# facebookresearch/param

Measured on AMD Instinct MI355X. Metric: EmbeddingBag lookups/s + achieved HBM GB/s; all-to-all bus-BW at 1/2/4/8 GPU, higher is better.
Workload: dtype f32

## Files before the change

param_amd/csrc/capi.hip:

```cpp
#include <atomic>
#include <cstdio>
#include <cstdlib>
#include <string>

#include "common.h"

namespace pm {
hipError_t launch_embbag_fwd_qrows(const KParams& p, int bits, int out_dtype, int max_dim, int unroll, hipStream_t stream);
hipError_t launch_embbag_fwd_qmixed(const KParams& p, const int32_t* table_bits, int out_dtype, int max_dim, int unroll, hipStream_t stream);
}

namespace {

thread_local std::string g_last_error;

std::atomic<int> g_unroll{0};
std::atomic<int> g_bags_per_block{0};
std::atomic<int> g_xcd_affine{-1};
std::atomic<int> g_nt_loads{-1};
std::atomic<int> g_stage_out{-1};
std::atomic<int> g_flat_target{-1};
std::atomic<int> g_flat_grid{-1};
constexpr int kDefaultRowPolicy = 3;

int fail(int code, const std::string& msg) {
    g_last_error = msg;
    return code;
}

int hip_fail(hipError_t rc, const char* what) {
    return fail(PM_ERR_HIP, std::string(what) + ": " + hipGetErrorString(rc));
}

const pm::FwdEnv& fwd_env() {
    static const pm::FwdEnv e = [] {
        auto num = [](const char* name, int dflt) { const char* v = getenv(name); return v ? atoi(v) : dflt; };
        pm::FwdEnv r;
        const char* st = getenv("PARAM_AMD_FWD_STAGE");
        r.stage = (st && st[0] == '0') ? 0 : 1;
        r.flat = num("PARAM_AMD_FWD_FLAT", r.flat);
        r.flat_maxl = num("PARAM_AMD_FLAT_MAXL", r.flat_maxl);
        r.flat_target = num("PARAM_AMD_FLAT_TARGET", r.flat_target);
        r.flat_bags = num("PARAM_AMD_FLAT_BAGS", r.flat_bags);
        r.tile_major = num("PARAM_AMD_FWD_TILE_MAJOR", r.tile_major);
        r.flat_compact = num("PARAM_AMD_FLAT_COMPACT", r.flat_compact);
        return r;
    }();
    return e;
}

pm::PlanKnobs current_knobs() {
    constexpr auto relaxed = std::memory_order_relaxed;
    pm::TuningSetters s;
    s.unroll = g_unroll.load(relaxed);
    s.bags_per_block = g_bags_per_block.load(relaxed);
    s.xcd_affine = g_xcd_affine.load(relaxed);
    s.nt_loads = g_nt_loads.load(relaxed);
    s.stage_out = g_stage_out.load(relaxed);
    s.flat_grid = g_flat_grid.load(relaxed);
    s.flat_target = g_flat_target.load(relaxed);
    return pm::resolve_knobs(s, fwd_env());
}

bool dtype_is_weight(int d) { return d == PM_F32 || d == PM_BF16 || d == PM_F16; }

const char* const kNoSortRecorded = "no sort has been recorded for this workspace";

enum class PlanKind { base, forward, quantized, padded, padded16 };

int validate_request(const pm_embbag_batch* op, int elem_dtype, const pm::PlanKnobs& knobs, pm::PlanShape* shape = nullptr);
void fill_params(const pm_embbag_batch* op, const pm::LaunchPlan& plan, pm::KParams& p);

pm::LaunchPlan plan_of(const pm_embbag_batch& op, const pm::PlanShape& shape, const pm::PlanKnobs& knobs, PlanKind kind) {
    return kind == PlanKind::forward     ? pm::plan_forward(op, shape, knobs)
           : kind == PlanKind::quantized ? pm::plan_quantized(op, shape, knobs)
           : kind == PlanKind::padded    ? pm::plan_padded(op, shape, knobs, 4)
           : kind == PlanKind::padded16  ? pm::plan_padded(op, shape, knobs, 2)
                                         : pm::plan_base(op, shape, knobs);
}

int make_params(const pm_embbag_batch* op, int elem_dtype, pm::KParams& p, PlanKind kind = PlanKind::base, int* unroll = nullptr) {
// ... 43 lines not shown
}

void fill_params(const pm_embbag_batch* op, const pm::LaunchPlan& plan, pm::KParams& p) {
    p.tables = op->tables;
    p.rows = op->rows;
    p.dims = op->dims;
    p.out_offsets = op->out_offsets;
    p.indices = op->indices;
    p.offsets = op->offsets;
    p.psw = op->per_sample_weights;
    p.io = nullptr;
    p.out_stride = op->out_stride;
    p.B = op->batch;
    p.N = op->num_indices;
    p.bag_begin = op->bag_begin;
    p.bag_count = op->bag_count;
    p.T = op->num_tables;
    p.idx64 = op->index_dtype == PM_I64 ? 1 : 0;
    p.alpha = 1.0f;
    p.gblk_shift = op->grad_block_shift > 0 ? op->grad_block_shift : 31;
    p.gblk_extra = op->grad_block_shift > 0 ? op->grad_block_extra : 0;
    p.out_bits = 0;
    p.tiles_per_table = plan.tiles_per_table;
    p.bags_per_block = plan.bags_per_block;
    p.idx_cap = plan.idx_cap;
    p.xcd_affine = plan.xcd_affine;
    p.nt_loads = plan.nt_loads;
    p.ordered = plan.ordered;
    p.stage_out = plan.stage_out;
    p.stage_bags = plan.stage_bags;
    p.flat_bags = plan.flat_bags;
    p.flat_target = plan.flat_target;
    p.flat_compact = plan.flat_compact;
}

int plan_fail(pm::PlanStatus st, const char* kind, bool sequence = false) {
    switch (st) {
        case pm::PlanStatus::ok: return PM_OK;
        case pm::PlanStatus::none:
            if (sequence)
                return fail(PM_ERR_INVALID, "pm_embseq_sort_indices has not been called for this request on this workspace (same indices / "
                                            "offsets pointers, batch and bag slice as the sort's)");
            return fail(PM_ERR_INVALID, "pm_embbag_sort_indices has not been called for this request on this workspace (same indices / "
                                        "offsets pointers, batch, bag slice and weights as the sort's)");
        case pm::PlanStatus::two_phase:
            return fail(PM_ERR_INVALID, std::string("the request was sorted for a two-phase scatter-add apply; ") + kind + " Adagrad needs "
                                        "pm_embbag_sort_indices (phases = 1)");
        case pm::PlanStatus::relabelled:
            return fail(PM_ERR_INVALID, "the sort on this workspace was relabelled by pm_embbag_sparse_grad_count (its keys hold slots, not "
                                        "rows): sort the request again");
        case pm::PlanStatus::not_complete_segmented:
            return fail(PM_ERR_UNSUPPORTED, "the sparse gradient needs the complete one-phase segmented sort: sort with pm_embbag_sort_indices "
                                            "(sort_impl 0)");
        case pm::PlanStatus::low_digit_order:
            return fail(PM_ERR_UNSUPPORTED, "the sparse gradient needs rows in ascending order within a table: sort mode 1 orders them by "
                                            "their low digit first (pm_set_sort_tuning 0, 2 or 3)");
        case pm::PlanStatus::sequence_sort:
            return fail(PM_ERR_INVALID, "the sort on this workspace is a sequence sort (pm_embseq_sort_indices: its values are lookup positions, "
                                        "not bags): only pm_embseq_bwd_sorted* may follow it; sort the request with pm_embbag_sort_indices");
        case pm::PlanStatus::pooled_sort:
            return fail(PM_ERR_INVALID, "the sort on this workspace is a pooled sort (pm_embbag_sort_indices: its values are bags, not lookup "
                                        "positions): a sequence apply needs pm_embseq_sort_indices");
        case pm::PlanStatus::already_counted:
            return fail(PM_ERR_INVALID, "pm_embbag_sparse_grad_count has been called for this sort already: sort the request again");
        default: return fail(PM_ERR_INVALID, "pm_embbag_sparse_grad needs pm_embbag_sparse_grad_count on this sort first");
    }
// ... 77 lines not shown

int pm_abi_version(void) { return PM_ABI_VERSION; }

const char* pm_build_info(void) {
    return "libparam_amd gfx950 (CDNA4, wave64) hip " __VERSION__;
}

const char* pm_last_error(void) { return g_last_error.c_str(); }

int pm_set_tuning(int32_t unroll, int32_t bags_per_block, int32_t xcd_affine, int32_t nt_loads) {
    if (unroll != 0 && unroll != 1 && unroll != 2 && unroll != 3 && unroll != 4 && unroll != 6 && unroll != 8)
        return fail(PM_ERR_INVALID, "unroll must be 0, 1, 2, 3, 4, 6 or 8");
    if (bags_per_block < 0) return fail(PM_ERR_INVALID, "bags_per_block must be >= 0");
    g_unroll.store(unroll);
    g_bags_per_block.store(bags_per_block);
    g_xcd_affine.store(xcd_affine);
    g_nt_loads.store(nt_loads);
    return PM_OK;
}

int pm_set_forward_tuning(int32_t stage_out, int32_t flat_grid, int32_t flat_target) {
    if (stage_out < -1 || stage_out > 1) return fail(PM_ERR_INVALID, "stage_out must be -1, 0 or 1");
    if (flat_grid < -1 || flat_grid > (1 << 20)) return fail(PM_ERR_INVALID, "flat_grid must be -1 (default), 0, 1 or a workgroup count up to 2^20");
    if (flat_target < -1 || flat_target == 0 || flat_target > 4096) return fail(PM_ERR_INVALID, "flat_target must be -1 (default) or 1 .. 4096");
    g_stage_out.store(stage_out);
    g_flat_grid.store(flat_grid);
    g_flat_target.store(flat_target);
    return PM_OK;
}

int pm_embbag_plan(const pm_embbag_batch* op, int32_t kind, int32_t out[12]) {
    if (kind < PM_PLAN_BASE || kind > PM_PLAN_PADDED16) return fail(PM_ERR_INVALID, "kind must be PM_PLAN_BASE .. PM_PLAN_PADDED16");
    if (!out) return fail(PM_ERR_INVALID, "out is NULL");
    static_assert(sizeof(pm::LaunchPlan) == 12 * sizeof(int32_t), "the query copies the twelve members in their order");
    const pm::PlanKnobs knobs = current_knobs();
    pm::PlanShape shape;
    const int rc = validate_request(op, op ? op->weight_dtype : -1, knobs, &shape);
    if (rc != PM_OK) return rc;
    constexpr PlanKind kinds[] = {PlanKind::base, PlanKind::forward, PlanKind::quantized, PlanKind::padded, PlanKind::padded16};
    const pm::LaunchPlan p = plan_of(*op, shape, knobs, kinds[kind]);
    const int32_t v[12] = {p.tiles_per_table, p.bags_per_block, p.idx_cap, p.xcd_affine, p.nt_loads, p.ordered,
                           p.stage_out, p.stage_bags, p.flat_bags, p.flat_target, p.flat_compact, p.unroll};
    for (int i = 0; i < 12; ++i) out[i] = v[i];
    return PM_OK;
}

int pm_embedding_gather_plan(const pm_embbag_batch* op, int64_t out[8]) {
    if (!out) return fail(PM_ERR_INVALID, "out is NULL");
    const pm::PlanKnobs knobs = current_knobs();
    const int rc = validate_request(op, op ? op->weight_dtype : -1, knobs);
    if (rc != PM_OK) return rc;
    const pm::GatherPlan g = pm::plan_gather(*op, op->weight_dtype, knobs);
    const int64_t v[8] = {g.vec, g.group_lanes, g.tile, g.col_passes, g.unroll, g.lds_borders, g.xcd_contiguous, g.grid};
    for (int i = 0; i < 8; ++i) out[i] = v[i];
    return PM_OK;
}

int pm_set_backward_tuning(int32_t sort_impl, int32_t order, int32_t xcd_affine, int32_t max_phases) {
    if (sort_impl < -1 || sort_impl > 2 || order < -1 || order > 1 || xcd_affine < -1 || xcd_affine > 1)
        return fail(PM_ERR_INVALID, "sort_impl must be -1 .. 2, order / xcd_affine -1, 0 or 1");
#ifndef PM_ALTERNATES
    if (sort_impl > 0)
        return fail(PM_ERR_UNSUPPORTED, "sort_impl 1 (rocPRIM) and 2 (round 2's LSD sort) exist in the alternates build only "
                                        "(libparam_amd_alt.so: make -C param_amd/csrc alt)");
#endif
    if (max_phases != -1 && max_phases != 1 && max_phases != 2) return fail(PM_ERR_INVALID, "max_phases must be -1, 1 or 2");
    pm::set_backward_tuning(sort_impl, order, xcd_affine, max_phases);
// ... 940 lines not shown
```

param_amd/csrc/common.h:

```cpp
#pragma once

#include <hip/hip_runtime.h>
#include <stdint.h>

#include <string>
#include <type_traits>

#include "param_amd.h"
#include "launch_plan.h"

namespace pm {

constexpr int kWave = 64;

typedef uint32_t u32x4 __attribute__((ext_vector_type(4)));
typedef float f32x4 __attribute__((ext_vector_type(4)));

#define PM_GLOBAL __attribute__((address_space(1)))
template <typename T>
__device__ __forceinline__ const PM_GLOBAL T* as_global(const void* p) { return (const PM_GLOBAL T*)(p); }
template <typename T>
__device__ __forceinline__ PM_GLOBAL T* as_global(void* p) { return (PM_GLOBAL T*)(p); }

struct KParams {
    const void* const* tables;
    const int64_t* rows;
    const int32_t* dims;
    const int64_t* out_offsets;
    const void* indices;
    const void* offsets;
    const float* psw;
    float* io;
    int64_t out_stride;
    int64_t B;
    int64_t N;
    int64_t bag_begin;
    int64_t bag_count;
    int32_t T;
    int32_t tiles_per_table;
    int32_t bags_per_block;
    int32_t idx_cap;
    int32_t idx64;
    int32_t xcd_affine;
    int32_t nt_loads;
    int32_t ordered;
    int32_t stage_out;
    int32_t stage_bags;
    int32_t out_bits;
    int32_t flat_bags;
    int32_t flat_target;
    int32_t flat_compact;
    int32_t gblk_shift;
    int64_t gblk_extra;
    float alpha;
};

__device__ __forceinline__ int64_t grad_bag_offset(int64_t bag, int64_t out_stride, int shift, int64_t extra) {
    int64_t o = bag * out_stride;
    if (__builtin_expect(extra != 0, 0)) o += (bag >> shift) * extra;
    return o;
}

__device__ __forceinline__ int64_t load_index(const void* p, int64_t i, int idx64) {
    return idx64 ? as_global<int64_t>(p)[i] : static_cast<int64_t>(as_global<int32_t>(p)[i]);
}

__device__ __forceinline__ int64_t bag_start_or_end(const KParams& p, int64_t g) {
    const int64_t TB = static_cast<int64_t>(p.T) * p.B;
    return (g < TB) ? load_index(p.offsets, g, p.idx64) : p.N;
}

__device__ __forceinline__ int xcd_contiguous_tile(int bid, int total) {
    const int q = total / kXcds, r = total % kXcds, x = bid % kXcds;
    return x * q + (x < r ? x : r) + bid / kXcds;
}

__device__ __forceinline__ void block_to_tile(const KParams& p, int& t, int& tile, int bid = blockIdx.x) {
    if (p.xcd_affine == 3) {
        const int g = xcd_contiguous_tile(bid, p.T * p.tiles_per_table);
        t = g / p.tiles_per_table;
        tile = g % p.tiles_per_table;
    } else if (p.xcd_affine == 2) {
        t = bid % p.T;
        tile = bid / p.T;
    } else if (p.xcd_affine) {
        const int xcd = bid % kXcds;
        const int slot = bid / kXcds;
        t = xcd + kXcds * (slot / p.tiles_per_table);
        tile = slot % p.tiles_per_table;
    } else {
        t = bid / p.tiles_per_table;
        tile = bid % p.tiles_per_table;
    }
}

__host__ __device__ inline size_t tile_idx_offset(int bags_per_block) {
    return (static_cast<size_t>(bags_per_block + 2) / 2 * 2) * sizeof(int64_t);
}
__host__ __device__ inline size_t tile_lds_bytes(int bags_per_block, int idx_cap, bool weighted) {
    return tile_idx_offset(bags_per_block) + static_cast<size_t>(idx_cap) * 4 * (weighted ? 2 : 1);
}

template <bool WEIGHTED>
__device__ __forceinline__ bool stage_tile_at(const KParams& p, int t, int64_t bag0, int nb, char* smem,
                                              int64_t*& s_off, int32_t*& s_idx, float*& s_w) {
    const int64_t g0 = static_cast<int64_t>(t) * p.B + bag0;

    s_off = reinterpret_cast<int64_t*>(smem);
    s_idx = reinterpret_cast<int32_t*>(smem + tile_idx_offset(p.bags_per_block));
    s_w = reinterpret_cast<float*>(s_idx + p.idx_cap);

    for (int i = threadIdx.x; i <= nb; i += kBlock) s_off[i] = bag_start_or_end(p, g0 + i);
    __syncthreads();
    const int64_t base = s_off[0];
    const int64_t cnt = s_off[nb] - base;
    const bool staged = cnt <= p.idx_cap;
    if (staged) {
        for (int i = threadIdx.x; i < static_cast<int>(cnt); i += kBlock) {
            s_idx[i] = static_cast<int32_t>(load_index(p.indices, base + i, p.idx64));
            if (WEIGHTED) s_w[i] = as_global<float>(p.psw)[base + i];
        }
        __syncthreads();
    }
    return staged;
}

// ... 259 lines not shown
```

param_amd/csrc/embbag_fwd.hip:

```cpp
#include <type_traits>

#include "common.h"
#include "fwd_elem.h"
#include "rowquant.inc"

namespace pm {
namespace {

using namespace fwd;

__device__ __forceinline__ float shfl_min(float v, int width) {
    for (int m = width / 2; m >= 1; m >>= 1) v = fminf(v, __shfl_xor(v, m, width));
    return v;
}
__device__ __forceinline__ float shfl_max(float v, int width) {
    for (int m = width / 2; m >= 1; m >>= 1) v = fmaxf(v, __shfl_xor(v, m, width));
    return v;
}

template <int BITS>
__device__ __forceinline__ void fused_rows_burst(const float* s_out, int nb, int D, uint8_t* qout, int64_t row0, int64_t rows_per_bag) {
    int gq = 4;
    while (gq * 8 < D) gq *= 2;
    const int lane = threadIdx.x % gq;
    const int c0 = lane * 4, c1 = (gq + lane) * 4;
    const bool has0 = c0 < D, has1 = c1 < D;
    const int64_t rb = rq::row_bytes(D, BITS);
    for (int r0 = 0; r0 < nb; r0 += kBlock / gq) {
        const int bg = r0 + threadIdx.x / gq;
        const bool live = bg < nb;
        const float* src = s_out + static_cast<size_t>(live ? bg : 0) * D;
        const f32x4 a = has0 ? *reinterpret_cast<const f32x4*>(src + c0) : f32x4{0, 0, 0, 0};
        const f32x4 b = has1 ? *reinterpret_cast<const f32x4*>(src + c1) : f32x4{0, 0, 0, 0};
        float mn, mx;
        rq::row_min_max(a, b, has0, has1, mn, mx);
        mn = shfl_min(mn, gq);
// ... 6 lines not shown

__device__ __forceinline__ void quantized_burst(const KParams& p, const float* s_out, int nb, int D, int64_t bag0, int64_t out_off) {
    uint8_t* qout = reinterpret_cast<uint8_t*>(p.io);
    const int64_t rows_per_bag = p.out_stride / D;
    const int64_t row0 = bag0 * rows_per_bag + out_off / D;
    switch (p.out_bits) {
        case 16: {
            typedef uint32_t u32x2 __attribute__((ext_vector_type(2)));
            const int q = D / 4;
            for (int i = threadIdx.x; i < nb * q; i += kBlock) {
                const int bg = i / q, c4 = i % q;
                const f32x4 v = *reinterpret_cast<const f32x4*>(s_out + static_cast<size_t>(bg) * D + c4 * 4);
                u32x2 o;
                o.x = rq::half_bits(v.x) | (static_cast<uint32_t>(rq::half_bits(v.y)) << 16);
                o.y = rq::half_bits(v.z) | (static_cast<uint32_t>(rq::half_bits(v.w)) << 16);
                __builtin_nontemporal_store(o, reinterpret_cast<u32x2*>(qout + (row0 + bg * rows_per_bag) * 2 * D) + c4);
            }
            break;
        }
        case 8: fused_rows_burst<8>(s_out, nb, D, qout, row0, rows_per_bag); break;
        case 4: fused_rows_burst<4>(s_out, nb, D, qout, row0, rows_per_bag); break;
        default: fused_rows_burst<2>(s_out, nb, D, qout, row0, rows_per_bag); break;
    }
}

template <typename WT, int G, int UNROLL, bool WEIGHTED, bool ORDERED, bool STAGE>
__global__ void __launch_bounds__(kBlock) embbag_fwd_kernel(const KParams p) {
    constexpr int VEC = Elem<WT>::kVec;
    constexpr int NG = kBlock / G;
    extern __shared__ __attribute__((aligned(16))) char smem[];
    __shared__ int s_next;

    int t, tile;
    block_to_tile(p, t, tile);
    if (t >= p.T) return;
    const int64_t bag0 = p.bag_begin + static_cast<int64_t>(tile) * p.bags_per_block;
    const int64_t left_bags = p.bag_begin + p.bag_count - bag0;
    const int nb = left_bags < p.bags_per_block ? static_cast<int>(left_bags) : p.bags_per_block;
    if (threadIdx.x == 0) s_next = NG;

    int64_t* s_off;
    int32_t* s_idx;
    float* s_w;
    const bool staged = stage_tile_at<WEIGHTED>(p, t, bag0, nb, smem, s_off, s_idx, s_w);
    const int64_t base = s_off[0];
    __shared__ uint16_t s_ord[ORDERED ? 1024 : 1];
    if (ORDERED) {
        if (nb <= kWave) {
            if (threadIdx.x < kWave) {
                const int i = threadIdx.x;
                int64_t len = i < nb ? s_off[i + 1] - s_off[i] : -1;
                if (len > 0x7fffffffffffLL) len = 0x7fffffffffffLL;
                uint64_t key = (static_cast<uint64_t>(len + 1) << 16) | static_cast<uint64_t>(0xffff - i);
#pragma unroll
                for (int k = 2; k <= kWave; k <<= 1) {
#pragma unroll
                    for (int j = k >> 1; j > 0; j >>= 1) {
                        const uint64_t other = __shfl_xor(key, j, kWave);
                        const bool take_max = ((i & k) == 0) == ((i & j) == 0);
                        key = take_max ? (key > other ? key : other) : (key < other ? key : other);
                    }
                }
                if (i < nb) s_ord[i] = static_cast<uint16_t>(0xffff - (key & 0xffff));
            }
        } else {
            for (int i = threadIdx.x; i < nb; i += kBlock) {
                const int64_t li = s_off[i + 1] - s_off[i];
                int rank = 0;
                for (int j = 0; j < nb; ++j) {
                    const int64_t lj = s_off[j + 1] - s_off[j];
                    rank += (lj > li) || (lj == li && j < i);
// ... 71 lines not shown
                        }
                    }
                }

                if (STAGE && stage) {
                    f32x4* o4 = reinterpret_cast<f32x4*>(s_out + static_cast<size_t>(bg) * D + c);
#pragma unroll
                    for (int k = 0; k < VEC; k += 4) o4[k / 4] = f32x4{acc[k], acc[k + 1], acc[k + 2], acc[k + 3]};
                } else {
                    f32x4* o4 = reinterpret_cast<f32x4*>(orow + c);
#pragma unroll
                    for (int k = 0; k < VEC; k += 4) {
                        f32x4 v = {acc[k], acc[k + 1], acc[k + 2], acc[k + 3]};
                        __builtin_nontemporal_store(v, o4 + k / 4);
                    }
                }
            }
        };
        if (staged) pool(std::true_type{}); else pool(std::false_type{});
        int nxt = 0;
        if (lig == 0) nxt = atomicAdd(&s_next, 1);
        slot = __shfl(nxt, 0, G);
    }
    if (STAGE && stage) {
        __syncthreads();
        if (p.out_bits == 0) {
            const int q = D / 4;
            if ((q & (q - 1)) != 0) burst_rows<false>(s_out, out_t, bag0, p.out_stride, nb, D);
            else burst_rows<true>(s_out, out_t, bag0, p.out_stride, nb, D);
        } else {
            quantized_burst(p, s_out, nb, D, bag0, p.out_offsets[t]);
        }
    }
}


__host__ __device__ inline size_t flat_tables_offset(const KParams& p, bool weighted) {
    return (tile_lds_bytes(p.bags_per_block, p.idx_cap, weighted) + static_cast<size_t>(p.stage_bags) * p.stage_out * sizeof(float) + 15) / 16 * 16;
}

template <typename WT, int G, int UNROLL, bool WEIGHTED>
__global__ void __launch_bounds__(kBlock) embbag_fwd_flat_kernel(const KParams p) {
    constexpr int VEC = Elem<WT>::kVec;
    extern __shared__ __attribute__((aligned(16))) char smem[];
    int* const s_pref = reinterpret_cast<int*>(smem + flat_tables_offset(p, WEIGHTED));
    uint16_t* const s_bags = reinterpret_cast<uint16_t*>(s_pref + p.T + 1);

    auto geometry = [&](int t, int& D, int& g, int& bags) {
        D = p.dims[t];
        g = kBlock / p.flat_bags;
        if (g < 1) g = 1;
        while (g < G && g * VEC < D) g <<= 1;
        const int NG = kBlock / g;
        const int64_t g0 = static_cast<int64_t>(t) * p.B + p.bag_begin;
        const int64_t lo = bag_start_or_end(p, g0), hi = bag_start_or_end(p, g0 + p.bag_count);
        const int64_t avg = p.bag_count > 0 ? (hi - lo + p.bag_count - 1) / p.bag_count : 1;
        bags = static_cast<int>(p.flat_target / (avg > 0 ? avg : 1));
        bags = bags > p.flat_bags ? p.flat_bags : bags;
        bags = bags / NG * NG;
        if (bags < NG) bags = NG;
    };

    auto do_tile = [&](int t, int tile, int D, int g, int bags) {
        const int NG = kBlock / g;
        const int64_t bag0 = p.bag_begin + static_cast<int64_t>(tile) * bags;
        const int64_t left_bags = p.bag_begin + p.bag_count - bag0;
// ... 106 lines not shown
                running += __shfl(v, kWave - 1, kWave);
            }
            if (threadIdx.x == 0) s_pref[0] = 0;
        }
        __syncthreads();
    }
    const int total = compact ? s_pref[p.T] : static_cast<int>(blockIdx.x) + 1;
    const int step = compact ? static_cast<int>(gridDim.x) : 1;
    for (int v = blockIdx.x; v < total; v += step) {
        int t, tile, D, g, bags;
        if (compact) {
            int lo = 0, hi = p.T;
            while (hi - lo > 1) {
                const int mid = (lo + hi) >> 1;
                if (s_pref[mid] <= v) lo = mid; else hi = mid;
            }
            t = lo;
            tile = v - s_pref[t];
            D = p.dims[t];
            g = kBlock / p.flat_bags;
            if (g < 1) g = 1;
            while (g < G && g * VEC < D) g <<= 1;
            bags = s_bags[t];
        } else {
            block_to_tile(p, t, tile);
            if (t >= p.T) return;
            geometry(t, D, g, bags);
        }
        do_tile(t, tile, D, g, bags);
        if (compact) __syncthreads();
    }
}

template <typename WT, int G, int UNROLL>
hipError_t launch_w(const KParams& p, hipStream_t stream) {
    const bool weighted = p.psw != nullptr;
    int grid = p.T * p.tiles_per_table;
    size_t lds = tile_lds_bytes(p.bags_per_block, p.idx_cap, weighted);
    if (p.flat_bags > 0) {
        lds += static_cast<size_t>(p.stage_bags) * p.stage_out * sizeof(float);
        if (p.flat_compact > 0) {
            lds = flat_tables_offset(p, weighted) + static_cast<size_t>(p.T + 1) * 4 + static_cast<size_t>(p.T) * 2;
            if (p.flat_compact < grid) grid = p.flat_compact;
        }
        dispatch_bool(weighted, [&](auto w) {
            hipLaunchKernelGGL((embbag_fwd_flat_kernel<WT, G, UNROLL, decltype(w)::value>), dim3(grid), dim3(kBlock), lds, stream, p);
        });
        return hipGetLastError();
    }
#define PM_FWD(W_, O_, S_) hipLaunchKernelGGL((embbag_fwd_kernel<WT, G, UNROLL, W_, O_, S_>), dim3(grid), dim3(kBlock), lds, stream, p)
    if (p.stage_out && !p.ordered) {
        lds += static_cast<size_t>(p.bags_per_block) * p.stage_out * sizeof(float);
        if (weighted) PM_FWD(true, false, true); else PM_FWD(false, false, true);
    } else if (weighted) { if (p.ordered) PM_FWD(true, true, false); else PM_FWD(true, false, false); }
    else { if (p.ordered) PM_FWD(false, true, false); else PM_FWD(false, false, false); }
#undef PM_FWD
    return hipGetLastError();
}

template <typename WT, int G>
hipError_t launch_u(const KParams& p, int unroll, hipStream_t stream) {
    switch (unroll) {
        case 1: return launch_w<WT, G, 1>(p, stream);
        case 2: return launch_w<WT, G, 2>(p, stream);
        case 3: return launch_w<WT, G, 3>(p, stream);
        case 4: return launch_w<WT, G, 4>(p, stream);
        case 6: return launch_w<WT, G, 6>(p, stream);
        default: return launch_w<WT, G, 8>(p, stream);
    }
}

template <typename WT>
hipError_t launch_g(const KParams& p, int max_dim, int unroll, hipStream_t stream) {
    return dispatch_group_lanes(group_lanes(max_dim, Elem<WT>::kVec),
                                [&](auto g) { return launch_u<WT, decltype(g)::value>(p, unroll, stream); });
}

}

hipError_t launch_embbag_fwd(const KParams& p, int weight_dtype, int max_dim, int unroll,
                             hipStream_t stream) {
    switch (weight_dtype) {
        case PM_F32: return launch_g<float>(p, max_dim, unroll, stream);
        case PM_BF16: return launch_g<bf16_t>(p, max_dim, unroll, stream);
        default: return launch_g<f16_t>(p, max_dim, unroll, stream);
    }
}

}
```

param_amd/csrc/launch_plan.h:

```cpp
#pragma once

#include <stdint.h>

#include "param_amd.h"

namespace pm {

constexpr int kBlock = 256;
constexpr int kXcds = 8;

inline int group_lanes(int max_dim, int vec) {
    int need = (max_dim + vec - 1) / vec;
    int g = 8;
    while (g < need && g < 64) g <<= 1;
    return g;
}

constexpr int kDefaultUnroll = 2;
constexpr int kBurstBytes = 16384;
constexpr int64_t kMaxGrid = 0x7fffffffLL;

struct FwdEnv {
    int stage = 1;
    int flat = 1;
    int flat_maxl = 0;
    int flat_target = 256;
    int flat_bags = 256;
    int tile_major = -1;
    int flat_compact = 1;
};
struct TuningSetters {
    int unroll = 0, bags_per_block = 0, xcd_affine = -1, nt_loads = -1;
    int stage_out = -1, flat_grid = -1, flat_target = -1;
};
struct PlanKnobs {
    int unroll;
    int bags_per_block;
    int xcd_affine;
    int nt_loads;
    int stage;
    int flat;
    int flat_maxl;
    int flat_target;
    int flat_bags;
    int flat_grid;
    int tile_major;
};
static inline PlanKnobs resolve_knobs(const TuningSetters& s, const FwdEnv& e) {
    PlanKnobs k;
    k.unroll = s.unroll;
    k.bags_per_block = s.bags_per_block;
    k.xcd_affine = s.xcd_affine;
    k.nt_loads = s.nt_loads;
    k.stage = s.stage_out >= 0 ? s.stage_out : e.stage;
    k.flat = e.flat;
    k.flat_maxl = e.flat_maxl;
    k.flat_target = s.flat_target > 0 ? s.flat_target : e.flat_target;
    if (k.flat_target < 1) k.flat_target = 1;
    k.flat_bags = e.flat_bags;
    k.flat_grid = s.flat_grid >= 0 ? s.flat_grid : e.flat_compact;
    k.tile_major = e.tile_major;
    return k;
}

struct LaunchPlan {
    int32_t tiles_per_table, bags_per_block, idx_cap, xcd_affine, nt_loads, ordered;
    int32_t stage_out, stage_bags, flat_bags, flat_target, flat_compact;
    int32_t unroll;
};

struct PlanShape {
    int vec;
    int G, NG;
    int64_t total_bags;
    int64_t avg_l;
    bool even;
    bool uneven;
    int base_tile;
};

static inline int64_t ceil_div(int64_t a, int64_t b) { return (a + b - 1) / b; }
static inline int64_t round256(int64_t n) { return (n + 255) / 256 * 256; }
static inline int64_t index_tile(int64_t bags, int64_t avg_l, int64_t floor) {
    const int64_t cap = round256(2 * bags * avg_l);
    return cap < floor ? floor : cap;
}
static inline int flat_bag_cap(int knob, int floor, int NG) { return knob < floor ? floor : (knob > 1024 ? 1024 : knob / NG * NG); }
static inline int burst_tile(int bpb, int NG, int max_dim, int elem_bytes) {
    while (bpb > NG && static_cast<int64_t>(bpb) * max_dim * elem_bytes > kBurstBytes) bpb /= 2;
    return bpb;
}

static inline int tile_bags(const pm_embbag_batch& op, const PlanShape& s, const PlanKnobs& k) {
    const int NG = s.NG;
    int bpb = k.bags_per_block;
    if (bpb <= 0) {
        bpb = 4 * NG;
        if (s.total_bags > 0 && op.num_indices < 12 * s.total_bags) bpb = NG;
        const int64_t want_blocks = 256 * 8;
        while (bpb > NG && op.num_tables * ceil_div(op.bag_count, bpb) < want_blocks) bpb /= 2;
    }
// ... 95 lines not shown
    if (p.flat_bags <= 0 || op.num_tables > 1024 || k.flat_grid <= 0) return p;
    const int64_t n_slice = op.batch > 0 ? ceil_div(op.num_indices * op.bag_count, op.batch) : 0;
    const int64_t by_lookups = ceil_div(n_slice, p.flat_target);
    const int64_t by_bags = op.num_tables * ceil_div(op.bag_count, p.flat_bags);
    int64_t est = (by_lookups > by_bags ? by_lookups : by_bags) * 5 / 4 + op.num_tables;
    if (est < 1024) est = 1024;
    if (est > (1 << 20)) est = 1 << 20;
    p.flat_compact = k.flat_grid > 1 ? k.flat_grid : static_cast<int32_t>(est);
    return p;
}

static inline LaunchPlan with_tile_major(const pm_embbag_batch& op, const PlanShape& s, const PlanKnobs& k, LaunchPlan p) {
    if (p.xcd_affine != 1 && op.num_tables > 1 && k.tile_major > 0 && s.uneven) p.xcd_affine = 2;
    return p;
}

static inline int small_request_unroll(const pm_embbag_batch& op, const PlanShape& s, const LaunchPlan& p) {
    if (p.flat_bags > 0 || p.ordered) return kDefaultUnroll;
    const int64_t wgs = static_cast<int64_t>(op.num_tables) * p.tiles_per_table;
    const int64_t avg_l = s.total_bags > 0 ? op.num_indices / s.total_bags : 0;
    if (wgs > 384) return kDefaultUnroll;
    return avg_l >= 8 ? 8 : (avg_l >= 4 ? 4 : kDefaultUnroll);
}

static inline LaunchPlan forward_geometry(const pm_embbag_batch& op, const PlanShape& s, const PlanKnobs& k) {
    LaunchPlan p = plan_base(op, s, k);
    p = with_burst_buffer(op, s, k, p);
    p = with_short_bag_flat_walk(op, s, k, p);
    p = with_mixed_dims(op, s, k, p);
    p = with_compact_grid(op, k, p);
    return with_tile_major(op, s, k, p);
}

static inline LaunchPlan plan_forward(const pm_embbag_batch& op, const PlanShape& s, const PlanKnobs& k) {
    LaunchPlan p = forward_geometry(op, s, k);
    p.unroll = k.unroll != 0 ? k.unroll : small_request_unroll(op, s, p);
    return p;
}
static inline LaunchPlan plan_forward(const pm_embbag_batch& op, int elem_dtype, const PlanKnobs& k) {
    return plan_forward(op, plan_shape(op, elem_dtype, k), k);
}

static inline LaunchPlan plan_quantized(const pm_embbag_batch& op, const PlanShape& s, const PlanKnobs& k) {
    LaunchPlan p = forward_geometry(op, s, k);
    if (p.flat_bags > 0) {
        p.bags_per_block = p.stage_bags;
        p.flat_bags = 0;
    }
    p.unroll = k.unroll != 0 ? k.unroll : kDefaultUnroll;
    return p;
}
static inline LaunchPlan plan_quantized(const pm_embbag_batch& op, int elem_dtype, const PlanKnobs& k) {
    return plan_quantized(op, plan_shape(op, elem_dtype, k), k);
}

static inline LaunchPlan plan_padded(const pm_embbag_batch& op, const PlanShape& s, const PlanKnobs& k, int out_bytes) {
    LaunchPlan p = plan_base(op, s, k);
    if (k.bags_per_block <= 0) p.bags_per_block = burst_tile(p.bags_per_block, s.NG, op.max_dim, out_bytes);
    p.tiles_per_table = static_cast<int32_t>(ceil_div(op.bag_count, p.bags_per_block));
    p.stage_out = (k.stage && static_cast<int64_t>(p.bags_per_block) * op.max_dim * out_bytes <= kBurstBytes) ? op.max_dim : 0;
    p.stage_bags = p.bags_per_block;
    if (s.even) {
        const int64_t need = index_tile(p.bags_per_block, s.avg_l, 512);
        if (need < p.idx_cap) p.idx_cap = static_cast<int32_t>(need);
    }
    p.ordered = 0;
    return p;
}
static inline LaunchPlan plan_padded(const pm_embbag_batch& op, int elem_dtype, const PlanKnobs& k, int out_bytes) {
    return plan_padded(op, plan_shape(op, elem_dtype, k), k, out_bytes);
// ... 30 lines not shown
        const int64_t need = index_tile(p.bags_per_block, s.avg_l, 512);
        if (need < p.idx_cap) p.idx_cap = static_cast<int32_t>(need);
    }
    p.ordered = 0;
    p.nt_loads = 0;
    const int u = k.unroll != 0 ? k.unroll : kQrowsUnroll;
    p.unroll = u >= 4 ? 4 : 2;
    return p;
}
static inline LaunchPlan plan_qrows(const pm_embbag_batch& op, int bits, const PlanKnobs& k, int out_bytes) {
    return plan_qrows(op, qrows_shape(op, bits, k), k, out_bytes);
}

constexpr int kQmixedLaneColumns = 8;
static inline PlanShape qmixed_shape(const pm_embbag_batch& op, const PlanKnobs& k) { return lane_columns_shape(op, kQmixedLaneColumns, k); }
static inline LaunchPlan plan_qmixed(const pm_embbag_batch& op, const PlanShape& s, const PlanKnobs& k, int out_bytes) { return plan_qrows(op, s, k, out_bytes); }
static inline LaunchPlan plan_qmixed(const pm_embbag_batch& op, const PlanKnobs& k, int out_bytes) { return plan_qmixed(op, qmixed_shape(op, k), k, out_bytes); }

constexpr int kGatherUnroll = 8;
constexpr int kGatherLdsBorders = kBlock;
struct GatherPlan {
    int32_t vec;
    int32_t group_lanes;
    int32_t tile;
    int32_t col_passes;
    int32_t unroll;
    int32_t lds_borders;
    int32_t xcd_contiguous;
    int64_t grid;
};
constexpr int64_t gather_block_tile(int64_t bid, int64_t total, bool xcd_contiguous) {
    return !xcd_contiguous ? bid : (bid % kXcds) * (total / kXcds) + ((bid % kXcds) < (total % kXcds) ? (bid % kXcds) : (total % kXcds)) + bid / kXcds;
}
static inline GatherPlan plan_gather(const pm_embbag_batch& op, int elem_dtype, const PlanKnobs& k) {
    GatherPlan g = {};
    g.vec = (elem_dtype == PM_F32) ? 4 : 8;
    g.group_lanes = group_lanes(op.max_dim, g.vec);
    g.tile = kBlock;
    g.col_passes = static_cast<int32_t>(ceil_div(op.max_dim, static_cast<int64_t>(g.group_lanes) * g.vec));
    const int u = k.unroll != 0 ? k.unroll : kGatherUnroll;
    g.unroll = u >= 8 ? 8 : (u >= 4 ? 4 : (u >= 2 ? 2 : 1));
    g.lds_borders = op.num_tables + 1 <= kGatherLdsBorders ? 1 : 0;
    g.xcd_contiguous = (op.num_tables > 1 && k.xcd_affine != 0) ? 1 : 0;
    g.grid = ceil_div(op.num_indices, g.tile);
    return g;
}

constexpr int kQgatherUnroll = 8;
static inline GatherPlan plan_gather_qrows(const pm_embbag_batch& op, int bits, const PlanKnobs& k) {
    GatherPlan g = {};
    g.vec = qrows_lane_columns(bits);
    g.group_lanes = group_lanes(op.max_dim, g.vec);
    g.tile = kBlock;
    g.col_passes = static_cast<int32_t>(ceil_div(op.max_dim, static_cast<int64_t>(g.group_lanes) * g.vec));
    const int u = k.unroll != 0 ? k.unroll : kQgatherUnroll;
    g.unroll = u >= 8 ? 8 : (u >= 4 ? 4 : (u >= 2 ? 2 : 1));
    g.lds_borders = op.num_tables + 1 <= kGatherLdsBorders ? 1 : 0;
    g.xcd_contiguous = (op.num_tables > 1 && k.xcd_affine != 0) ? 1 : 0;
    g.grid = ceil_div(op.num_indices, g.tile);
    return g;
}

static inline GatherPlan plan_gather_qmixed(const pm_embbag_batch& op, const PlanKnobs& k) {
    GatherPlan g = {};
    g.vec = kQmixedLaneColumns;
    g.group_lanes = group_lanes(op.max_dim, g.vec);
// ... 12 lines not shown
```

param_amd/csrc/pm_experiments.h:

```cpp
#pragma once

#ifdef PM_EXPERIMENTS
#include <hip/hip_runtime.h>
#include <stdint.h>
namespace pm {
namespace exp {
constexpr int kTraceSlots = 8;
constexpr int kTraceWgs = 1 << 15;
namespace {
__device__ unsigned long long g_trace[kTraceWgs * kTraceSlots];
}
__device__ __forceinline__ void stamp(unsigned wg, int slot, bool drain) {
    if (drain) asm volatile("s_waitcnt vmcnt(0) lgkmcnt(0)" ::: "memory");
    if (threadIdx.x == 0 && wg < static_cast<unsigned>(kTraceWgs)) g_trace[wg * kTraceSlots + slot] = __builtin_amdgcn_s_memrealtime();
}
}
}
#define PM_STAMP(wg, slot) pm::exp::stamp((wg), (slot), false)
#define PM_STAMP_DRAINED(wg, slot) pm::exp::stamp((wg), (slot), true)
#define PM_DEFINE_TRACE_READER(fn)                                                                                                      \
    extern "C" int fn(unsigned long long* out, int words, int clear) {                                                                  \
        const size_t all = sizeof(unsigned long long) * pm::exp::kTraceWgs * pm::exp::kTraceSlots;                                      \
        const size_t bytes = sizeof(unsigned long long) * static_cast<size_t>(words);                                                   \
        if (bytes > all) return -1;                                                                                                     \
        if (hipDeviceSynchronize() != hipSuccess) return -2;                                                                            \
        if (out && bytes && hipMemcpyFromSymbol(out, HIP_SYMBOL(pm::exp::g_trace), bytes) != hipSuccess) return -3;                     \
        if (clear) {                                                                                                                    \
            void* p = nullptr;                                                                                                          \
            if (hipGetSymbolAddress(&p, HIP_SYMBOL(pm::exp::g_trace)) != hipSuccess || hipMemset(p, 0, all) != hipSuccess) return -4;   \
        }                                                                                                                               \
        return 0;                                                                                                                       \
    }
#else
#define PM_STAMP(wg, slot) ((void)0)
#define PM_STAMP_DRAINED(wg, slot) ((void)0)
#define PM_DEFINE_TRACE_READER(fn)
#endif
```

Before: 22.17 billion.

## Split tail-round forward tiles across extra workgroups to shorten drain

Adds a drain-split scheduling mode for the staged, unordered forward EmbeddingBag kernel. When the per-XCD tile slots do not divide evenly into the resident workgroup count, the tiles of the last partial round are split into up to four sub-tiles, each with fewer bags, and extra blocks are launched to cover them. The aim is to reduce tail idle time while the final wave drains. The cost is an occupancy query on first launch (cached per kernel), more blocks, and per-bag overheads on smaller sub-tiles. Experiment tracing hooks and per-call env rereads are added only under PM_EXPERIMENTS.

```diff
diff --git a/param_amd/csrc/capi.hip b/param_amd/csrc/capi.hip
--- a/param_amd/csrc/capi.hip
+++ b/param_amd/csrc/capi.hip
@@ -33,7 +33,7 @@
 }
 
 const pm::FwdEnv& fwd_env() {
-    static const pm::FwdEnv e = [] {
+    const auto read = [] {
         auto num = [](const char* name, int dflt) { const char* v = getenv(name); return v ? atoi(v) : dflt; };
         pm::FwdEnv r;
         const char* st = getenv("PARAM_AMD_FWD_STAGE");
@@ -44,9 +44,18 @@
         r.flat_bags = num("PARAM_AMD_FLAT_BAGS", r.flat_bags);
         r.tile_major = num("PARAM_AMD_FWD_TILE_MAJOR", r.tile_major);
         r.flat_compact = num("PARAM_AMD_FLAT_COMPACT", r.flat_compact);
+        r.drain_split = num("PARAM_AMD_FWD_DRAIN_SPLIT", r.drain_split);
+        r.round_wgs = num("PARAM_AMD_FWD_ROUND_WGS", r.round_wgs);
         return r;
-    }();
+    };
+#ifdef PM_EXPERIMENTS
+    static thread_local pm::FwdEnv again;
+    again = read();
+    return again;
+#else
+    static const pm::FwdEnv e = read();
     return e;
+#endif
 }
 
 pm::PlanKnobs current_knobs() {
@@ -156,6 +165,8 @@
     p.flat_bags = plan.flat_bags;
     p.flat_target = plan.flat_target;
     p.flat_compact = plan.flat_compact;
+    p.round_wgs = plan.round_wgs;
+    p.drain_split = plan.drain_split;
 }
 
 int plan_fail(pm::PlanStatus st, const char* kind, bool sequence = false) {
@@ -299,7 +310,7 @@
 int pm_embbag_plan(const pm_embbag_batch* op, int32_t kind, int32_t out[12]) {
     if (kind < PM_PLAN_BASE || kind > PM_PLAN_PADDED16) return fail(PM_ERR_INVALID, "kind must be PM_PLAN_BASE .. PM_PLAN_PADDED16");
     if (!out) return fail(PM_ERR_INVALID, "out is NULL");
-    static_assert(sizeof(pm::LaunchPlan) == 12 * sizeof(int32_t), "the query copies the twelve members in their order");
+    static_assert(offsetof(pm::LaunchPlan, unroll) == 11 * sizeof(int32_t), "the query copies the twelve reported members in their order");
     const pm::PlanKnobs knobs = current_knobs();
     pm::PlanShape shape;
     const int rc = validate_request(op, op ? op->weight_dtype : -1, knobs, &shape);
diff --git a/param_amd/csrc/common.h b/param_amd/csrc/common.h
--- a/param_amd/csrc/common.h
+++ b/param_amd/csrc/common.h
@@ -53,6 +53,8 @@
     int32_t gblk_shift;
     int64_t gblk_extra;
     float alpha;
+    int32_t round_wgs;
+    int32_t drain_split;
 };
 
 __device__ __forceinline__ int64_t grad_bag_offset(int64_t bag, int64_t out_stride, int shift, int64_t extra) {
@@ -92,6 +94,20 @@
         t = bid / p.tiles_per_table;
         tile = bid % p.tiles_per_table;
     }
+}
+
+__device__ __forceinline__ void block_to_tile(const KParams& p, int& t, int& tile, int& part, int& parts, int bid = blockIdx.x) {
+    if (p.round_wgs > 0) {
+        const BlockTile b = drain_block_tile(bid, p.T, p.tiles_per_table, p.round_wgs, p.drain_split);
+        t = b.table;
+        tile = b.tile;
+        part = b.part;
+        parts = b.parts;
+        return;
+    }
+    part = 0;
+    parts = 1;
+    block_to_tile(p, t, tile, bid);
 }
 
 __host__ __device__ inline size_t tile_idx_offset(int bags_per_block) {
diff --git a/param_amd/csrc/embbag_fwd.hip b/param_amd/csrc/embbag_fwd.hip
--- a/param_amd/csrc/embbag_fwd.hip
+++ b/param_amd/csrc/embbag_fwd.hip
@@ -1,7 +1,11 @@
+#include <map>
+#include <mutex>
+#include <tuple>
 #include <type_traits>
 
 #include "common.h"
 #include "fwd_elem.h"
+#include "pm_experiments.h"
 #include "rowquant.inc"
 
 namespace pm {
@@ -74,11 +78,27 @@
     __shared__ int s_next;
 
     int t, tile;
-    block_to_tile(p, t, tile);
-    if (t >= p.T) return;
-    const int64_t bag0 = p.bag_begin + static_cast<int64_t>(tile) * p.bags_per_block;
+    int64_t bag0;
+    int run_bags = p.bags_per_block;
+    if (STAGE && !ORDERED) {
+        int part, parts;
+        block_to_tile(p, t, tile, part, parts);
+        if (t >= p.T) return;
+        bag0 = p.bag_begin + static_cast<int64_t>(tile) * p.bags_per_block;
+        if (parts > 1) {
+            run_bags = p.bags_per_block / parts;
+            bag0 += static_cast<int64_t>(part) * run_bags;
+            if (bag0 >= p.bag_begin + p.bag_count) return;
+        }
+    } else {
+        block_to_tile(p, t, tile);
+        if (t >= p.T) return;
+        bag0 = p.bag_begin + static_cast<int64_t>(tile) * p.bags_per_block;
+    }
+    PM_STAMP(blockIdx.x, 0);
+    PM_STAMP_VALUE(blockIdx.x, 2, (static_cast<unsigned long long>(PM_XCC_ID()) << 32) | static_cast<unsigned>(t));
     const int64_t left_bags = p.bag_begin + p.bag_count - bag0;
-    const int nb = left_bags < p.bags_per_block ? static_cast<int>(left_bags) : p.bags_per_block;
+    const int nb = left_bags < run_bags ? static_cast<int>(left_bags) : run_bags;
     if (threadIdx.x == 0) s_next = NG;
 
     int64_t* s_off;
@@ -216,6 +236,7 @@
             quantized_burst(p, s_out, nb, D, bag0, p.out_offsets[t]);
         }
     }
+    PM_STAMP_DRAINED(blockIdx.x, 1);
 }
 
 
@@ -388,8 +409,47 @@
     }
 }
 
+int resident_wgs_per_xcd(const void* kernel, size_t lds, hipStream_t stream) {
+    static std::mutex mu;
+    static std::map<std::tuple<int, const void*, size_t>, int> known;
+    int dev = 0;
+    if (hipGetDevice(&dev) != hipSuccess) return 0;
+    const auto key = std::make_tuple(dev, kernel, lds);
+    std::lock_guard<std::mutex> lock(mu);
+    const auto it = known.find(key);
+    if (it != known.end()) return it->second;
+    hipStreamCaptureStatus capturing = hipStreamCaptureStatusNone;
+    if (hipStreamIsCapturing(stream, &capturing) != hipSuccess) {
+        (void)hipGetLastError();
+        return 0;
+    }
+    if (capturing != hipStreamCaptureStatusNone) return 0;
+    int per_cu = 0, cus = 0;
+    if (hipOccupancyMaxActiveBlocksPerMultiprocessor(&per_cu, kernel, kBlock, lds) != hipSuccess ||
+        hipDeviceGetAttribute(&cus, hipDeviceAttributeMultiprocessorCount, dev) != hipSuccess) {
+        (void)hipGetLastError();
+        return 0;
+    }
+    const int r = per_cu * (cus / kXcds);
+    known.emplace(key, r);
+    return r;
+}
+
+void apply_drain_split(KParams& p, int& grid, const void* kernel, size_t lds, hipStream_t stream) {
+    const int want_split = p.drain_split, given = p.round_wgs;
+    p.round_wgs = p.drain_split = 0;
+    if (want_split <= 1 || p.xcd_affine != 1) return;
+    const int R = given > 0 ? given : resident_wgs_per_xcd(kernel, lds, stream);
+    const DrainSplit o = resolve_drain_split(p.T, p.tiles_per_table, R, want_split);
+    p.round_wgs = o.round_wgs;
+    p.drain_split = o.drain_split;
+    grid += o.extra_blocks;
+}
+
 template <typename WT, int G, int UNROLL>
-hipError_t launch_w(const KParams& p, hipStream_t stream) {
+hipError_t launch_w(const KParams& request, hipStream_t stream) {
+    KParams p = request;
+    if (p.flat_bags > 0 || !p.stage_out || p.ordered) p.round_wgs = p.drain_split = 0;
     const bool weighted = p.psw != nullptr;
     int grid = p.T * p.tiles_per_table;
     size_t lds = tile_lds_bytes(p.bags_per_block, p.idx_cap, weighted);
@@ -405,12 +465,20 @@
         return hipGetLastError();
     }
 #define PM_FWD(W_, O_, S_) hipLaunchKernelGGL((embbag_fwd_kernel<WT, G, UNROLL, W_, O_, S_>), dim3(grid), dim3(kBlock), lds, stream, p)
+#define PM_FWD_ADDR(W_, O_, S_) reinterpret_cast<const void*>(&embbag_fwd_kernel<WT, G, UNROLL, W_, O_, S_>)
     if (p.stage_out && !p.ordered) {
         lds += static_cast<size_t>(p.bags_per_block) * p.stage_out * sizeof(float);
-        if (weighted) PM_FWD(true, false, true); else PM_FWD(false, false, true);
+        if (weighted) {
+            apply_drain_split(p, grid, PM_FWD_ADDR(true, false, true), lds, stream);
+            PM_FWD(true, false, true);
+        } else {
+            apply_drain_split(p, grid, PM_FWD_ADDR(false, false, true), lds, stream);
+            PM_FWD(false, false, true);
+        }
     } else if (weighted) { if (p.ordered) PM_FWD(true, true, false); else PM_FWD(true, false, false); }
     else { if (p.ordered) PM_FWD(false, true, false); else PM_FWD(false, false, false); }
 #undef PM_FWD
+#undef PM_FWD_ADDR
     return hipGetLastError();
 }
 
@@ -444,3 +512,5 @@
 }
 
 }
+
+PM_DEFINE_TRACE_READER(pm_experiment_trace_fwd)
diff --git a/param_amd/csrc/launch_plan.h b/param_amd/csrc/launch_plan.h
--- a/param_amd/csrc/launch_plan.h
+++ b/param_amd/csrc/launch_plan.h
@@ -28,6 +28,8 @@
     int flat_bags = 256;
     int tile_major = -1;
     int flat_compact = 1;
+    int drain_split = 4;
+    int round_wgs = 0;
 };
 struct TuningSetters {
     int unroll = 0, bags_per_block = 0, xcd_affine = -1, nt_loads = -1;
@@ -45,6 +47,8 @@
     int flat_bags;
     int flat_grid;
     int tile_major;
+    int drain_split;
+    int round_wgs;
 };
 static inline PlanKnobs resolve_knobs(const TuningSetters& s, const FwdEnv& e) {
     PlanKnobs k;
@@ -60,6 +64,8 @@
     k.flat_bags = e.flat_bags;
     k.flat_grid = s.flat_grid >= 0 ? s.flat_grid : e.flat_compact;
     k.tile_major = e.tile_major;
+    k.drain_split = e.drain_split;
+    k.round_wgs = e.round_wgs;
     return k;
 }
 
@@ -67,6 +73,8 @@
     int32_t tiles_per_table, bags_per_block, idx_cap, xcd_affine, nt_loads, ordered;
     int32_t stage_out, stage_bags, flat_bags, flat_target, flat_compact;
     int32_t unroll;
+    int32_t round_wgs;
+    int32_t drain_split;
 };
 
 struct PlanShape {
@@ -228,10 +236,19 @@
     return with_tile_major(op, s, k, p);
 }
 
+static inline LaunchPlan with_drain_split(const PlanShape& s, const PlanKnobs& k, LaunchPlan p) {
+    if (p.xcd_affine != 1 || p.stage_out <= 0 || p.ordered || p.flat_bags > 0 || !s.even) return p;
+    int split = 1;
+    while (split * 2 <= k.drain_split && split * 2 * s.NG <= p.bags_per_block && p.bags_per_block % (split * 2) == 0) split *= 2;
+    p.drain_split = split;
+    p.round_wgs = split > 1 && k.round_wgs > 0 ? k.round_wgs : 0;
+    return p;
+}
+
 static inline LaunchPlan plan_forward(const pm_embbag_batch& op, const PlanShape& s, const PlanKnobs& k) {
     LaunchPlan p = forward_geometry(op, s, k);
     p.unroll = k.unroll != 0 ? k.unroll : small_request_unroll(op, s, p);
-    return p;
+    return with_drain_split(s, k, p);
 }
 static inline LaunchPlan plan_forward(const pm_embbag_batch& op, int elem_dtype, const PlanKnobs& k) {
     return plan_forward(op, plan_shape(op, elem_dtype, k), k);
@@ -328,6 +345,35 @@
 constexpr int64_t gather_block_tile(int64_t bid, int64_t total, bool xcd_contiguous) {
     return !xcd_contiguous ? bid : (bid % kXcds) * (total / kXcds) + ((bid % kXcds) < (total % kXcds) ? (bid % kXcds) : (total % kXcds)) + bid / kXcds;
 }
+struct BlockTile {
+    int32_t table, tile;
+    int32_t part, parts;
+};
+constexpr BlockTile drain_block_tile(int32_t bid, int32_t T, int32_t tiles_per_table, int32_t R, int32_t S) {
+    const int32_t main_grid = T * tiles_per_table;
+    const int32_t slots = T / kXcds * tiles_per_table;
+    const int32_t drain = S > 1 ? slots % R : 0;
+    int32_t xcd = bid % kXcds, slot = bid / kXcds, part = 0;
+    if (bid >= main_grid) {
+        const int32_t e = bid - main_grid;
+        xcd = e % kXcds;
+        slot = slots - drain + (e / kXcds) / (S - 1);
+        part = 1 + (e / kXcds) % (S - 1);
+    }
+    return BlockTile{xcd + kXcds * (slot / tiles_per_table), slot % tiles_per_table, part, slot >= slots - drain ? S : 1};
+}
+struct DrainSplit {
+    int32_t round_wgs, drain_split;
+    int32_t extra_blocks;
+};
+constexpr DrainSplit resolve_drain_split(int32_t T, int32_t tiles_per_table, int32_t R, int32_t want_split) {
+    if (R <= 0 || T % kXcds != 0 || tiles_per_table <= 0 || want_split <= 1) return DrainSplit{0, 0, 0};
+    const int64_t slots = static_cast<int64_t>(T / kXcds) * tiles_per_table;
+    const int64_t extra = kXcds * (slots % R) * (want_split - 1);
+    if (slots <= R || extra == 0 || static_cast<int64_t>(T) * tiles_per_table + extra > kMaxGrid) return DrainSplit{0, 0, 0};
+    return DrainSplit{R, want_split, static_cast<int32_t>(extra)};
+}
+
 static inline GatherPlan plan_gather(const pm_embbag_batch& op, int elem_dtype, const PlanKnobs& k) {
     GatherPlan g = {};
     g.vec = (elem_dtype == PM_F32) ? 4 : 8;
diff --git a/param_amd/csrc/pm_experiments.h b/param_amd/csrc/pm_experiments.h
--- a/param_amd/csrc/pm_experiments.h
+++ b/param_amd/csrc/pm_experiments.h
@@ -14,8 +14,13 @@
     if (drain) asm volatile("s_waitcnt vmcnt(0) lgkmcnt(0)" ::: "memory");
     if (threadIdx.x == 0 && wg < static_cast<unsigned>(kTraceWgs)) g_trace[wg * kTraceSlots + slot] = __builtin_amdgcn_s_memrealtime();
 }
+__device__ __forceinline__ void stamp_value(unsigned wg, int slot, unsigned long long v) {
+    if (threadIdx.x == 0 && wg < static_cast<unsigned>(kTraceWgs)) g_trace[wg * kTraceSlots + slot] = v;
 }
 }
+}
+#define PM_STAMP_VALUE(wg, slot, v) pm::exp::stamp_value((wg), (slot), (v))
+#define PM_XCC_ID() __builtin_amdgcn_s_getreg((3 << 11) | (0 << 6) | 20)
 #define PM_STAMP(wg, slot) pm::exp::stamp((wg), (slot), false)
 #define PM_STAMP_DRAINED(wg, slot) pm::exp::stamp((wg), (slot), true)
 #define PM_DEFINE_TRACE_READER(fn)                                                                                                      \
@@ -34,5 +39,6 @@
 #else
 #define PM_STAMP(wg, slot) ((void)0)
 #define PM_STAMP_DRAINED(wg, slot) ((void)0)
+#define PM_STAMP_VALUE(wg, slot, v) ((void)0)
 #define PM_DEFINE_TRACE_READER(fn)
 #endif
```

Result: faster. 22.47 billion, median of 6 (+1.4%).
